# chaofengc/FeMaSR

Measured on AMD Instinct MI355X. Metric: SR output megapixels/sec at x4 (128->512), higher is better.
Workload: dtype f32 (1x1 convs / nn.Linear: every fp32 operand split EXACTLY into three bf16 terms, six partial products, fp32 accumulation on the bf16 matrix pipe - closer to fp64 than the fp32 fmaf chain, bit-identical to the CPU oracle)

## Files before the change

femasr_amd/csrc/kernels_misc.hip:

```cpp
#include "common.h"
#include "detmath.h"
#include <stdlib.h>
#include <string.h>
#include <type_traits>

namespace {

__device__ __forceinline__ float4 ld4(const float *p) { return *reinterpret_cast<const float4 *>(p); }

__device__ __forceinline__ int xcd_remap_misc(int bid, int nblk)
{
    const int q = nblk >> 3, r = nblk & 7, xcd = bid & 7, within = bid >> 3;
    return (xcd < r ? xcd * (q + 1) : r * (q + 1) + (xcd - r) * q) + within;
}

__global__ void pad_nchw_to_nhwc_kernel(const float *__restrict__ in, int B, int C, int H, int W, int Hp, int Wp,
                                        float *__restrict__ out, size_t total)
{
    for (size_t i = blockIdx.x * (size_t)blockDim.x + threadIdx.x; i < total; i += (size_t)gridDim.x * blockDim.x) {
        const int c = (int)(i % C);
        size_t r = i / C;
        const int x = (int)(r % Wp);
        r /= Wp;
        const int y = (int)(r % Hp);
// ... 149 lines not shown
    const int slabs = C >> 5, cg = C >> 5;
    int b = blockIdx.x;
    const int slab = b % slabs;
    b /= slabs;
    const int tx = b % tilesX;
    b /= tilesX;
    const int ty = b % tilesY;
    const int n = b / tilesY;
    const float *xn = x + (size_t)n * H * W * C + slab * 32 + c31;
    double S = 0.0, SS = 0.0;
#pragma unroll
    for (int q = 0; q < 4; ++q) {
        double s = 0.0, ss = 0.0;
#pragma unroll
        for (int r = 0; r < 16; ++r) {
            const int m = 32 * q + 4 * h + (r & 3) + 8 * (r >> 2);
            const int y = 8 * ty + (m >> 4), xx = 16 * tx + (m & 15);
            if (y < H && xx < W) {
                const double d = (double)xn[((size_t)y * W + xx) * C];
                s = s + d;
                ss = __builtin_fma(d, d, ss);
            }
        }
        s = s + __shfl_xor(s, 32, 64);
        ss = ss + __shfl_xor(ss, 32, 64);
        for (int d = 1; d < cg; d <<= 1) {
            s = s + __shfl_xor(s, d, 64);
            ss = ss + __shfl_xor(ss, d, 64);
        }
        if (q == 0) { S = s; SS = ss; } else { S = S + s; SS = SS + ss; }
    }
    const int ch = slab * 32 + c31;
    if (lane < 32 && (ch & (cg - 1)) == 0) {
        double *dst = part + ((((size_t)n * tilesY + ty) * tilesX + tx) * 32 + ch / cg) * 2;
        dst[0] = S;
        dst[1] = SS;
    }
}

__global__ __launch_bounds__(64) void gn_finalize_partials_kernel(const double *__restrict__ part, int tiles, int H, int W, int C, int G,
                                                                  const float *__restrict__ gamma, const float *__restrict__ beta,
                                                                  float eps, float *__restrict__ a, float *__restrict__ b)
{
    const int n = blockIdx.x / G, g = blockIdx.x % G, lane = threadIdx.x, cg = C / G;
    const double *src = part + ((size_t)n * tiles * G + g) * 2;
    double S = 0.0, SS = 0.0;
    for (int t = lane; t < tiles; t += 64) {
        S += src[(size_t)t * G * 2];
        SS += src[(size_t)t * G * 2 + 1];
    }
#pragma unroll
    for (int sft = 32; sft >= 1; sft >>= 1) {
        S += __shfl_xor(S, sft, 64);
        SS += __shfl_xor(SS, sft, 64);
    }
    const double N = (double)H * (double)W * (double)cg;
    const double mean = S / N;
    double var = SS / N - mean * mean;
    if (var < 0.0) var = 0.0;
    const float rstd = 1.0f / sqrtf((float)var + eps);
    const float meanf = (float)mean;
    if (lane < cg) {
        const int c = g * cg + lane;
        const float ac = rstd * gamma[c];
        a[n * C + c] = ac;
        b[n * C + c] = __builtin_fmaf(-meanf, ac, beta[c]);
    }
}

__global__ void gn_silu_apply_kernel(const float *__restrict__ x, int C, long long hw, const float *__restrict__ a, const float *__restrict__ b,
                                     float *__restrict__ y, size_t total4)
{
    const int c4n = C >> 2;
    for (size_t i = blockIdx.x * (size_t)blockDim.x + threadIdx.x; i < total4; i += (size_t)gridDim.x * blockDim.x) {
        const int c4 = (int)(i % c4n);
        const size_t n = (i / c4n) / (size_t)hw;
        const float4 v = ld4(x + 4 * i), ga = ld4(a + n * C + 4 * c4), gb = ld4(b + n * C + 4 * c4);
        float4 o;
        o.x = det_silu(__builtin_fmaf(v.x, ga.x, gb.x));
        o.y = det_silu(__builtin_fmaf(v.y, ga.y, gb.y));
        o.z = det_silu(__builtin_fmaf(v.z, ga.z, gb.z));
        o.w = det_silu(__builtin_fmaf(v.w, ga.w, gb.w));
        *reinterpret_cast<float4 *>(y + 4 * i) = o;
    }
}

__device__ __forceinline__ float wave_tree_sum(float p)
{
#pragma unroll
    for (int s = 32; s >= 1; s >>= 1) p = p + __shfl_xor(p, s, 64);
    return p;
}

__global__ void ln_stats_kernel(const float *__restrict__ x, long long rows, float eps, float *__restrict__ stats)
{
    const long long row = (long long)blockIdx.x * (blockDim.x >> 6) + (threadIdx.x >> 6);
    if (row >= rows) return;
    const int lane = threadIdx.x & 63;
    const float4 v = ld4(x + row * 256 + lane * 4);
    float s = v.x;
    s = s + v.y;
    s = s + v.z;
    s = s + v.w;
    const float mean = wave_tree_sum(s) * (1.0f / 256.0f);
    float d = v.x - mean;
    float q = d * d;
    d = v.y - mean;
    q = __builtin_fmaf(d, d, q);
    d = v.z - mean;
    q = __builtin_fmaf(d, d, q);
    d = v.w - mean;
    q = __builtin_fmaf(d, d, q);
    const float var = wave_tree_sum(q) * (1.0f / 256.0f);
    if (lane == 0) {
        stats[2 * row] = mean;
        stats[2 * row + 1] = 1.0f / sqrtf(var + eps);
    }
}

__global__ void layernorm_kernel(const float *__restrict__ x, long long rows, const float *__restrict__ gamma,
                                 const float *__restrict__ beta, float eps, float *__restrict__ y)
{
    const long long row = (long long)blockIdx.x * (blockDim.x >> 6) + (threadIdx.x >> 6);
    if (row >= rows) return;
    const int lane = threadIdx.x & 63;
    const float4 v = ld4(x + row * 256 + lane * 4);
    float s = v.x;
    s = s + v.y;
    s = s + v.z;
    s = s + v.w;
    const float mean = wave_tree_sum(s) * (1.0f / 256.0f);
    float d = v.x - mean;
    float q = d * d;
    d = v.y - mean;
    q = __builtin_fmaf(d, d, q);
    d = v.z - mean;
    q = __builtin_fmaf(d, d, q);
    d = v.w - mean;
    q = __builtin_fmaf(d, d, q);
    const float var = wave_tree_sum(q) * (1.0f / 256.0f);
    const float rstd = 1.0f / sqrtf(var + eps);
    const float4 g = ld4(gamma + lane * 4), b = ld4(beta + lane * 4);
    float4 o;
    o.x = __builtin_fmaf((v.x - mean) * rstd, g.x, b.x);
    o.y = __builtin_fmaf((v.y - mean) * rstd, g.y, b.y);
    o.z = __builtin_fmaf((v.z - mean) * rstd, g.z, b.z);
    o.w = __builtin_fmaf((v.w - mean) * rstd, g.w, b.w);
    *reinterpret_cast<float4 *>(y + row * 256 + lane * 4) = o;
}

constexpr int ATT_HD = 32, ATT_N = 64;
typedef float att_f32x16 __attribute__((ext_vector_type(16)));

template <int UNITS>
__global__ __launch_bounds__(64, 2) void window_attention_reg_kernel(const float *__restrict__ qkv, int B, int H, int W, int C,
                                                                     int heads, int shift, const float *__restrict__ table,
                                                                     float *__restrict__ out, int total)
{
    __shared__ float Ts[UNITS][232];
    const int lane = threadIdx.x, c = lane & 31, hf = lane >> 5;
    const int nwx = W >> 3, nwy = H >> 3;
    struct Unit { int h, wx, wy, n; };
    auto unit_of = [&](int bid) {
        Unit g;
        g.h = bid % heads;
        bid /= heads;
        g.wx = bid % nwx;
        bid /= nwx;
        g.wy = bid % nwy;
        g.n = bid / nwy;
        return g;
    };
    Unit gs[UNITS];
    bool has[UNITS];
#pragma unroll
    for (int u = 0; u < UNITS; ++u) {
        const int bid = (int)blockIdx.x * UNITS + u;
        has[u] = bid < total;
        gs[u] = unit_of(has[u] ? bid : total - 1);
        for (int i = lane; i < 225; i += 64) Ts[u][i] = table[i * heads + gs[u].h];
    }
    const float scale = 0.17677669529663687f;
    auto rowtok = [&](const Unit &g, int iy) { int y = g.wy * 8 + iy + shift; if (y >= H) y -= H; return y * W; };
    auto coltok = [&](const Unit &g, int ix) { int x = g.wx * 8 + ix + shift; if (x >= W) x -= W; return x; };
    auto qb = [&](const Unit &g) { return qkv + (size_t)g.n * H * W * 3 * C + g.h * ATT_HD; };

    float ak[2][16], bq[2][16];
    auto load_qk = [&](const Unit &g) {
        const float *qbase = qb(g);
#pragma unroll
        for (int tI = 0; tI < 2; ++tI) {
            const int w = 32 * tI + c;
            const unsigned tok = (unsigned)(rowtok(g, w >> 3) + coltok(g, w & 7));
            const float *kp = qbase + tok * (unsigned)(3 * C) + C, *qp = qbase + tok * (unsigned)(3 * C);
#pragma unroll
            for (int d4 = 0; d4 < 8; ++d4) {
                const float4 kv = ld4(kp + 4 * d4), qv = ld4(qp + 4 * d4);
                ak[tI][2 * d4] = hf ? kv.y : kv.x;
                ak[tI][2 * d4 + 1] = hf ? kv.w : kv.z;
                bq[tI][2 * d4] = (hf ? qv.y : qv.x) * scale;
                bq[tI][2 * d4 + 1] = (hf ? qv.w : qv.z) * scale;
            }
        }
    };
    load_qk(gs[0]);
#pragma unroll
    for (int u = 0; u < UNITS; ++u) {
        if (!has[u]) break;
        const Unit g = gs[u];
        const float *qbase = qb(g);
        float *obase = out + (size_t)g.n * H * W * C + g.h * ATT_HD;
        const bool masked = shift > 0 && (g.wy == nwy - 1 || g.wx == nwx - 1);
        att_f32x16 sc[2][2];
#pragma unroll
        for (int tj = 0; tj < 2; ++tj)
#pragma unroll
            for (int ti = 0; ti < 2; ++ti)
#pragma unroll
                for (int r = 0; r < 16; ++r) sc[tj][ti][r] = 0.f;
#pragma unroll
        for (int st = 0; st < 16; ++st)
#pragma unroll
            for (int tj = 0; tj < 2; ++tj)
#pragma unroll
                for (int ti = 0; ti < 2; ++ti) sc[tj][ti] = __builtin_amdgcn_mfma_f32_32x32x2f32(ak[tj][st], bq[ti][st], sc[tj][ti], 0, 0, 0);

        float vf[2][16];
        {
            const float *vb = qbase + 2 * C + c;
            unsigned cto[4];
#pragma unroll
            for (int e = 0; e < 4; ++e) cto[e] = (unsigned)coltok(g, e + 4 * hf) * (unsigned)(3 * C);
#pragma unroll
            for (int tj = 0; tj < 2; ++tj)
#pragma unroll
                for (int r = 0; r < 16; ++r) {
                    const unsigned ro = (unsigned)__builtin_amdgcn_readfirstlane(rowtok(g, (r >> 2) + 4 * tj)) * (unsigned)(3 * C);
                    vf[tj][r] = vb[ro + cto[r & 3]];
                }
        }
        if (u + 1 < UNITS && has[u + 1 < UNITS ? u + 1 : u]) load_qk(gs[u + 1 < UNITS ? u + 1 : u]);
#pragma unroll
        for (int ti = 0; ti < 2; ++ti) {
            const int i = 32 * ti + c, iy = i >> 3, ix = i & 7;
            const int tb = (iy + 7) * 15 + ix + 7 - 4 * hf;
            unsigned rowdiff = 0, coldiff = 0;
            if (masked) {
                const int ysi = g.wy * 8 + iy, xsi = g.wx * 8 + ix;
                const int ryi = ysi < H - 8 ? 0 : (ysi < H - shift ? 1 : 2), rxi = xsi < W - 8 ? 0 : (xsi < W - shift ? 1 : 2);
#pragma unroll
                for (int q = 0; q < 8; ++q) {
                    const int ysj = g.wy * 8 + q, xsj = g.wx * 8 + q;
                    const int ryj = ysj < H - 8 ? 0 : (ysj < H - shift ? 1 : 2), rxj = xsj < W - 8 ? 0 : (xsj < W - shift ? 1 : 2);
                    rowdiff |= (ryj != ryi ? 1u : 0u) << q;
                    coldiff |= (rxj != rxi ? 1u : 0u) << q;
                }
                coldiff >>= 4 * hf;
            }
            float m = -INFINITY;
#pragma unroll
            for (int tj = 0; tj < 2; ++tj)
#pragma unroll
                for (int r = 0; r < 16; ++r) {
                    const int jy = (r >> 2) + 4 * tj, jxl = r & 3;
                    float a1 = sc[tj][ti][r] + Ts[u][tb - 15 * jy - jxl];
                    if (masked) a1 = a1 + ((((rowdiff >> jy) | (coldiff >> jxl)) & 1u) ? -100.0f : 0.0f);
                    sc[tj][ti][r] = a1;
                    m = a1 > m ? a1 : m;
                }
            {
                const float mo = __shfl_xor(m, 32, 64);
                m = mo > m ? mo : m;
            }
            float part = 0.f;
#pragma unroll
            for (int tj = 0; tj < 2; ++tj)
#pragma unroll
                for (int r = 0; r < 16; r += 2) {
                    const det_f32x2 e = det_expf2(det_f32x2{sc[tj][ti][r] - m, sc[tj][ti][r + 1] - m});
                    sc[tj][ti][r] = e[0];
                    sc[tj][ti][r + 1] = e[1];
                    part = part + e[0];
                    part = part + e[1];
                }
            const float other = __shfl_xor(part, 32, 64);
            const float rinv = 1.0f / (hf ? other + part : part + other);
#pragma unroll
            for (int tj = 0; tj < 2; ++tj) sc[tj][ti] = sc[tj][ti] * rinv;
        }

        att_f32x16 oc[2];
#pragma unroll
        for (int ti = 0; ti < 2; ++ti)
#pragma unroll
            for (int r = 0; r < 16; ++r) oc[ti][r] = 0.f;
#pragma unroll
        for (int tj = 0; tj < 2; ++tj)
#pragma unroll
            for (int r = 0; r < 16; ++r)
#pragma unroll
                for (int ti = 0; ti < 2; ++ti) oc[ti] = __builtin_amdgcn_mfma_f32_32x32x2f32(sc[tj][ti][r], vf[tj][r], oc[ti], 0, 0, 0);

        {
            float *ob = obase + c;
            unsigned cto[4];
#pragma unroll
            for (int e = 0; e < 4; ++e) cto[e] = (unsigned)coltok(g, e + 4 * hf) * (unsigned)C;
#pragma unroll
            for (int ti = 0; ti < 2; ++ti)
#pragma unroll
                for (int r = 0; r < 16; ++r) {
                    const unsigned ro = (unsigned)__builtin_amdgcn_readfirstlane(rowtok(g, (r >> 2) + 4 * ti)) * (unsigned)C;
                    ob[ro + cto[r & 3]] = oc[ti][r];
                }
        }
    }
}

__global__ void row_sqsum_kernel(const float *__restrict__ x, long long rows, int D, float *__restrict__ out)
{
    const long long r = (long long)blockIdx.x * blockDim.x + threadIdx.x;
    if (r >= rows) return;
    const float *p = x + r * D;
    float acc = 0.f;
    for (int c = 0; c < D; c += 4) {
        const float4 v = ld4(p + c);
        acc = __builtin_fmaf(v.x, v.x, acc);
        acc = __builtin_fmaf(v.y, v.y, acc);
        acc = __builtin_fmaf(v.z, v.z, acc);
        acc = __builtin_fmaf(v.w, v.w, acc);
    }
    out[r] = acc;
}

__global__ void vq_finalize_kernel(const float *__restrict__ z, long long M, int D, const float *__restrict__ cb,
                                   const float *__restrict__ part, int nblk, int n_e, long long *__restrict__ idx,
                                   float *__restrict__ zq)
{
    const long long row = (long long)blockIdx.x * (blockDim.x >> 6) + (threadIdx.x >> 6);
    if (row >= M) return;
    const int lane = threadIdx.x & 63;
    const float *pp = part + (size_t)row * nblk * 2;
    float bd = pp[0];
    int bi = __float_as_int(pp[1]);
    for (int b = 1; b < nblk; ++b) {
        const float d = pp[2 * b];
        const int i = __float_as_int(pp[2 * b + 1]);
        if (d < bd || (d == bd && i < bi)) { bd = d; bi = i; }
    }
    bi = bi < 0 ? 0 : (bi >= n_e ? n_e - 1 : bi);
    if (lane == 0) idx[row] = (long long)bi;
    const float *e = cb + (size_t)bi * D;
    const float *zr = z + (size_t)row * D;
    float *o = zq + (size_t)row * D;
    for (int c = lane * 4; c < D; c += 256) {
        const float4 zv = ld4(zr + c), ev = ld4(e + c);
        float4 r;
        r.x = zv.x + (ev.x - zv.x);
        r.y = zv.y + (ev.y - zv.y);
        r.z = zv.z + (ev.z - zv.z);
        r.w = zv.w + (ev.w - zv.w);
        *reinterpret_cast<float4 *>(o + c) = r;
    }
}

__global__ void codebook_gather_kernel(const long long *__restrict__ idx, long long M, int D, const float *__restrict__ cb,
                                       int n_e, float *__restrict__ zq)
{
    const long long row = (long long)blockIdx.x * (blockDim.x >> 6) + (threadIdx.x >> 6);
    if (row >= M) return;
    const int lane = threadIdx.x & 63;
    long long i = idx[row];
    i = i < 0 ? 0 : (i >= n_e ? n_e - 1 : i);
    for (int c = lane * 4; c < D; c += 256)
        *reinterpret_cast<float4 *>(zq + (size_t)row * D + c) = ld4(cb + (size_t)i * D + c);
}

__global__ void repack_oihw_kernel(const float *__restrict__ in, int O, int I, int kh, int kw, float *__restrict__ out,
                                   size_t total)
{
    const bool blocked = (I % 32) == 0;
    const int K = I * kh * kw, NT32 = (O + 31) / 32;
    for (size_t i = blockIdx.x * (size_t)blockDim.x + threadIdx.x; i < total; i += (size_t)gridDim.x * blockDim.x) {
        const int kk = (int)(i & 15), lane = (int)((i >> 4) & 63);
        const size_t rest = i >> 10;
        const int ntile = (int)(rest % NT32), q = (int)(rest / NT32);
        const int k = q * 32 + kk * 2 + (lane >> 5), o = ntile * 32 + (lane & 31);
        float v = 0.f;
        if (k < K && o < O) {
            int ci, x, y;
            if (blocked) {
                const int cl = k % 32;
                int r = k / 32;
                x = r % kw;
                r /= kw;
                y = r % kh;
                ci = (r / kh) * 32 + cl;
            } else {
                ci = k % I;
                const int r = k / I;
                x = r % kw;
                y = r / kw;
            }
            v = in[(((size_t)o * I + ci) * kh + y) * kw + x];
        }
        out[i] = v;
    }
}

__global__ void repack_up2_kernel(const float *__restrict__ in, int O, int I, float *__restrict__ out, size_t per_phase)
{
    const int K = I * 4, NT32 = (O + 31) / 32;
    for (size_t i = blockIdx.x * (size_t)blockDim.x + threadIdx.x; i < 4 * per_phase; i += (size_t)gridDim.x * blockDim.x) {
        const int ph = (int)(i / per_phase);
        const size_t e = i - (size_t)ph * per_phase;
        const int kk = (int)(e & 15), lane = (int)((e >> 4) & 63);
        const size_t rest = e >> 10;
        const int ntile = (int)(rest % NT32), q = (int)(rest / NT32);
        const int k = q * 32 + kk * 2 + (lane >> 5), o = ntile * 32 + (lane & 31);
        float v = 0.f;
        if (k < K && o < O) {
            const int a = ph >> 1, b = ph & 1;
            const int cl = k % 32, r = k / 32, tap = r & 3, ci = (r >> 2) * 32 + cl;
            const int ty = tap >> 1, tx = tap & 1;
            const int y0 = ty == 0 ? 0 : (a == 0 ? 1 : 2), y1 = ty == 0 ? (a == 0 ? 0 : 1) : 2;
            const int x0 = tx == 0 ? 0 : (b == 0 ? 1 : 2), x1 = tx == 0 ? (b == 0 ? 0 : 1) : 2;
            const float *w = in + ((size_t)o * I + ci) * 9;
            for (int ky = y0; ky <= y1; ++ky) {
                float row = w[ky * 3 + x0];
                for (int kx = x0 + 1; kx <= x1; ++kx) row = row + w[ky * 3 + kx];
                v = ky == y0 ? row : v + row;
            }
        }
        out[i] = v;
    }
}

__global__ void repack_compact_kernel(const float *__restrict__ in, int O, int I, int kh, int kw, float *__restrict__ out, size_t total)
{
    for (size_t i = blockIdx.x * (size_t)blockDim.x + threadIdx.x; i < total; i += (size_t)gridDim.x * blockDim.x) {
        const int o = (int)(i & 3), k = (int)(i >> 2);
        const int cl = k % 32;
        int r = k / 32;
        const int x = r % kw;
        r /= kw;
        const int y = r % kh, ci = (r / kh) * 32 + cl;
        out[i] = o < O ? in[(((size_t)o * I + ci) * kh + y) * kw + x] : 0.f;
    }
}

__global__ void image_u8_to_f32_kernel(const unsigned char *__restrict__ in, int H, int W, int swap_rb,
                                       float *__restrict__ out, size_t total)
{
    for (size_t i = blockIdx.x * (size_t)blockDim.x + threadIdx.x; i < total; i += (size_t)gridDim.x * blockDim.x) {
        const int x = (int)(i % W);
        size_t r = i / W;
        const int y = (int)(r % H);
        const int c = (int)(r / H);
        const int sc = swap_rb ? 2 - c : c;
        out[i] = (float)in[((size_t)y * W + x) * 3 + sc] / 255.0f;
    }
}

__global__ void image_f32_to_u8_kernel(const float *__restrict__ in, int H, int W, int swap_rb,
                                       unsigned char *__restrict__ out, size_t total)
{
    for (size_t i = blockIdx.x * (size_t)blockDim.x + threadIdx.x; i < total; i += (size_t)gridDim.x * blockDim.x) {
        const int c = (int)(i % 3);
// ... 154 lines not shown
}

typedef float probe_f32x16 __attribute__((ext_vector_type(16)));
__global__ __launch_bounds__(256) void clock_probe_kernel(int groups, float a, float b, unsigned long long *ticks)
{
    probe_f32x16 c0 = {0}, c1 = {0}, c2 = {0}, c3 = {0};
    a += (float)(threadIdx.x & 31) * 0.03125f;
    b += (float)((threadIdx.x >> 5) & 1) * 0.25f;
    const unsigned long long t0 = __builtin_readcyclecounter();
    for (int i = 0; i < groups; ++i) {
        c0 = __builtin_amdgcn_mfma_f32_32x32x2f32(a, b, c0, 0, 0, 0);
        c1 = __builtin_amdgcn_mfma_f32_32x32x2f32(a, b, c1, 0, 0, 0);
        c2 = __builtin_amdgcn_mfma_f32_32x32x2f32(a, b, c2, 0, 0, 0);
        c3 = __builtin_amdgcn_mfma_f32_32x32x2f32(a, b, c3, 0, 0, 0);
    }
    float s = 0.f;
    for (int r = 0; r < 16; ++r) s += c0[r] + c1[r] + c2[r] + c3[r];
    const unsigned long long t1 = __builtin_readcyclecounter();
    if ((threadIdx.x & 63) == 0) ticks[blockIdx.x * 4 + (threadIdx.x >> 6)] = (t1 - t0) + (s == 12345.678f ? 1ull : 0ull);
}

extern "C" {

int femasr_pad_nchw_to_nhwc(void *stream, const float *in, int B, int C, int H, int W, int Hp, int Wp, float *out)
{
    FEMASR_REQUIRE(in && out && B > 0 && C > 0 && H > 0 && W > 0, "pad: bad args");
    FEMASR_REQUIRE(Hp >= H && Wp >= W && Hp - H <= H && Wp - W <= W, "pad: mirror pad larger than the image (%d,%d)->(%d,%d)", H, W, Hp, Wp);
    const size_t total = (size_t)B * Hp * Wp * C;
    hipLaunchKernelGGL(pad_nchw_to_nhwc_kernel, dim3(grid_for(total)), dim3(256), 0, (hipStream_t)stream, in, B, C, H, W,
                       Hp, Wp, out, total);
    FEMASR_CHECK_HIP(hipGetLastError());
    return FEMASR_OK;
}

int femasr_pad_u8hwc_to_nhwc(void *stream, const uint8_t *in, int B, int H, int W, int swap_rb, int Hp, int Wp, float *out)
{
    FEMASR_REQUIRE(in && out && B > 0 && H > 0 && W > 0 && Hp >= H && Wp >= W && Hp <= 2 * H && Wp <= 2 * W, "pad_u8: bad args");
    const size_t total = (size_t)B * Hp * Wp * 3;
    hipLaunchKernelGGL(pad_u8hwc_to_nhwc_kernel, dim3(grid_for(total)), dim3(256), 0, (hipStream_t)stream, in, B, H, W, swap_rb, Hp, Wp, out, total);
    FEMASR_CHECK_HIP(hipGetLastError());
    return FEMASR_OK;
}

int femasr_crop_nhwc_to_u8hwc(void *stream, const float *in, int B, int Hs, int Ws, int Hc, int Wc, int swap_rb, uint8_t *out)
{
    FEMASR_REQUIRE(in && out && B > 0 && Hc > 0 && Wc > 0 && Hc <= Hs && Wc <= Ws, "crop_u8: bad args");
    const size_t total = (size_t)B * Hc * Wc * 3;
    hipLaunchKernelGGL(crop_nhwc_to_u8hwc_kernel, dim3(grid_for(total)), dim3(256), 0, (hipStream_t)stream, in, B, Hs, Ws, Hc, Wc, swap_rb, out, total);
    FEMASR_CHECK_HIP(hipGetLastError());
    return FEMASR_OK;
}

int femasr_crop_nhwc_to_nchw(void *stream, const float *in, int B, int Hs, int Ws, int C, int Hc, int Wc, float *out)
{
    FEMASR_REQUIRE(in && out && B > 0 && C > 0 && Hc > 0 && Wc > 0 && Hc <= Hs && Wc <= Ws, "crop: bad args");
    const size_t total = (size_t)B * C * Hc * Wc;
    hipLaunchKernelGGL(crop_nhwc_to_nchw_kernel, dim3(grid_for(total)), dim3(256), 0, (hipStream_t)stream, in, B, Hs, Ws,
                       C, Hc, Wc, out, total);
    FEMASR_CHECK_HIP(hipGetLastError());
    return FEMASR_OK;
}

size_t femasr_gn_scratch_bytes(int B, int H, int W, int C, int G)
{
    if (B <= 0 || H <= 0 || W <= 0 || G <= 0) return 0;
    if (G == 32 && femasr_gn_fusable(C)) return (size_t)B * ((H + 7) / 8) * ((W + 15) / 16) * 32 * 2 * sizeof(double);
    return (size_t)B * H * G * 2 * sizeof(double);
}

int femasr_gn_coeffs(void *stream, const float *x, int B, int H, int W, int C, int G, const float *gamma,
                     const float *beta, float eps, float *a, float *b, void *scratch)
{
    FEMASR_REQUIRE(x && gamma && beta && a && b && scratch, "gn_coeffs: null pointer");
    FEMASR_REQUIRE(B > 0 && H > 0 && W > 0 && G > 0 && C % G == 0, "gn_coeffs: bad shape C=%d G=%d", C, G);
    const int cg = C / G;
    hipStream_t s = (hipStream_t)stream;
    double *part = (double *)scratch;
    if (G == 32 && femasr_gn_fusable(C)) {
        const int tilesX = (W + 15) / 16, tilesY = (H + 7) / 8;
        hipLaunchKernelGGL(gn_tile_partials_kernel, dim3((unsigned)((size_t)B * tilesY * tilesX * (C / 32))), dim3(64), 0, s, x, H, W, C,
                           tilesX, tilesY, part);
        FEMASR_CHECK_HIP(hipGetLastError());
        return femasr_gn_coeffs_from_partials(stream, part, B, tilesX * tilesY, H, W, C, G, gamma, beta, eps, a, b);
    }
    const size_t total = (size_t)B * H * G;
    const dim3 grid((unsigned)((total + 255) / 256)), blk(256);
    if (cg == 8 && C % 4 == 0)
        hipLaunchKernelGGL(gn_rows_kernel<8>, grid, blk, 0, s, x, B, H, W, C, G, part);
    else if (cg == 4 && C % 4 == 0)
        hipLaunchKernelGGL(gn_rows_kernel<4>, grid, blk, 0, s, x, B, H, W, C, G, part);
    else if (cg == 2)
        hipLaunchKernelGGL(gn_rows_kernel<2>, grid, blk, 0, s, x, B, H, W, C, G, part);
    else
        hipLaunchKernelGGL(gn_rows_generic_kernel, grid, blk, 0, s, x, B, H, W, C, G, cg, part);
    FEMASR_CHECK_HIP(hipGetLastError());
    FEMASR_REQUIRE(G <= 256, "gn_coeffs: at most 256 groups");
    hipLaunchKernelGGL(gn_finalize_kernel, dim3((unsigned)B), dim3(256), (size_t)GN_SLAB * G * 2 * sizeof(double), s, part, B, H, H,
                       W, C, G, gamma, beta, eps, a, b);
    FEMASR_CHECK_HIP(hipGetLastError());
    return FEMASR_OK;
}

int femasr_gn_coeffs_from_partials(void *stream, const double *part, int B, int tiles, int H, int W, int C, int G,
                                   const float *gamma, const float *beta, float eps, float *a, float *b)
{
    FEMASR_REQUIRE(part && gamma && beta && a && b && B > 0 && tiles > 0 && H > 0 && W > 0, "gn_coeffs_from_partials: bad args");
    FEMASR_REQUIRE(G == 32 && C % G == 0, "gn_coeffs_from_partials: 32 groups");
    FEMASR_REQUIRE(C / G <= 64, "gn_coeffs_from_partials: at most 64 channels per group");
    hipLaunchKernelGGL(gn_finalize_partials_kernel, dim3((unsigned)(B * G)), dim3(64), 0, (hipStream_t)stream, part, tiles, H, W, C,
                       G, gamma, beta, eps, a, b);
    FEMASR_CHECK_HIP(hipGetLastError());
    return FEMASR_OK;
}

int femasr_gn_silu_apply(void *stream, const float *x, int B, int H, int W, int C, const float *a, const float *b, float *y)
{
    FEMASR_REQUIRE(x && a && b && y && B > 0 && H > 0 && W > 0 && C > 0 && (C % 4) == 0, "gn_silu_apply: bad args (C %% 4 == 0)");
    const size_t total4 = (size_t)B * H * W * (C / 4);
    hipLaunchKernelGGL(gn_silu_apply_kernel, dim3(grid_for(total4)), dim3(256), 0, (hipStream_t)stream, x, C, (long long)H * W, a, b, y, total4);
    FEMASR_CHECK_HIP(hipGetLastError());
    return FEMASR_OK;
}

int femasr_ln_stats(void *stream, const float *x, int64_t rows, int C, float eps, float *stats)
{
    FEMASR_REQUIRE(x && stats && rows > 0, "ln_stats: bad args");
    FEMASR_REQUIRE(C == 256, "ln_stats: only C == 256 (Swin embed_dim, femasr_arch.py:115) is built, got %d", C);
    hipLaunchKernelGGL(ln_stats_kernel, dim3((unsigned)((rows + 3) / 4)), dim3(256), 0, (hipStream_t)stream, x,
                       (long long)rows, eps, stats);
    FEMASR_CHECK_HIP(hipGetLastError());
    return FEMASR_OK;
}

int femasr_layernorm(void *stream, const float *x, int64_t rows, int C, const float *gamma, const float *beta, float eps, float *y)
{
    FEMASR_REQUIRE(x && y && gamma && beta && rows > 0, "layernorm: bad args");
    FEMASR_REQUIRE(C == 256, "layernorm: only C == 256 (Swin embed_dim, femasr_arch.py:115) is built, got %d", C);
    hipLaunchKernelGGL(layernorm_kernel, dim3((unsigned)((rows + 3) / 4)), dim3(256), 0, (hipStream_t)stream, x, (long long)rows,
                       gamma, beta, eps, y);
    FEMASR_CHECK_HIP(hipGetLastError());
    return FEMASR_OK;
}

int femasr_window_attention(void *stream, const float *qkv, int B, int H, int W, int C, int heads, int shift,
                            const float *table, float *out)
{
    FEMASR_REQUIRE(qkv && table && out && B > 0, "window_attention: bad args");
    FEMASR_REQUIRE(H % 8 == 0 && W % 8 == 0 && H >= 8 && W >= 8, "window_attention: H,W must be multiples of 8 (%d,%d)", H, W);
    FEMASR_REQUIRE(heads > 0 && heads <= 8 && C == heads * ATT_HD, "window_attention: head_dim must be 32, at most 8 heads (C=%d heads=%d)", C, heads);
    FEMASR_REQUIRE(shift >= 0 && shift < 8, "window_attention: bad shift %d", shift);
    FEMASR_REQUIRE((size_t)H * W * 3 * C < ((size_t)1 << 30), "window_attention: image too large for 32-bit offsets");
    const size_t total = (size_t)B * (H / 8) * (W / 8) * heads;
    FEMASR_REQUIRE(total < ((size_t)1 << 31), "window_attention: too many (window, head) units");
    hipLaunchKernelGGL(window_attention_reg_kernel<1>, dim3((unsigned)total), dim3(64), 0, (hipStream_t)stream, qkv, B, H, W, C, heads, shift, table,
                       out, (int)total);
    FEMASR_CHECK_HIP(hipGetLastError());
    return FEMASR_OK;
}

int femasr_row_sqsum(void *stream, const float *x, int64_t rows, int D, float *out)
{
    FEMASR_REQUIRE(x && out && rows > 0 && D > 0 && D % 4 == 0, "row_sqsum: bad args");
    hipLaunchKernelGGL(row_sqsum_kernel, dim3((unsigned)((rows + 63) / 64)), dim3(64), 0, (hipStream_t)stream, x,
                       (long long)rows, D, out);
    FEMASR_CHECK_HIP(hipGetLastError());
    return FEMASR_OK;
}

int femasr_vq(void *stream, const float *z, int64_t M, int D, const float *cb, const float *cbT, const float *ee,
              int n_e, int64_t *idx, float *zq, void *scratch)
{
    FEMASR_REQUIRE(z && cb && cbT && ee && idx && zq && scratch && M > 0, "vq: bad args");
    FEMASR_REQUIRE(D % 32 == 0 && n_e % 128 == 0, "vq: needs e_dim %% 32 == 0 and n_e %% 128 == 0 (D=%d n_e=%d)", D, n_e);
    FEMASR_REQUIRE(M < (1ll << 31) - 256, "vq: too many rows");
    hipStream_t s = (hipStream_t)stream;
    float *zz = (float *)scratch;
    float *part = zz + ((M + 63) / 64) * 64;
    const int nblk = n_e / 128;
    int rc = femasr_row_sqsum(stream, z, M, D, zz);
    if (rc) return rc;
    femasr_conv_args a{};
    a.in = z; a.B = 1; a.H = (int)M; a.W = 1; a.Cin = D; a.w = cbT; a.bias = nullptr; a.Cout = n_e;
    a.ksz = 1; a.stride = 1; a.pad = 0; a.up2 = 0; a.prologue = FEMASR_PRO_NONE; a.act = 0;
    a.Ho = (int)M; a.Wo = 1;
    conv_vq_epilogue ep{zz, ee, part, nblk};
    rc = femasr_conv2d_launch(s, &a, &ep, nullptr, nullptr);
    if (rc) return rc;
    hipLaunchKernelGGL(vq_finalize_kernel, dim3((unsigned)((M + 3) / 4)), dim3(256), 0, s, z, (long long)M, D, cb, part,
                       nblk, n_e, (long long *)idx, zq);
    FEMASR_CHECK_HIP(hipGetLastError());
    return FEMASR_OK;
}

int femasr_codebook_gather(void *stream, const int64_t *idx, int64_t M, int D, const float *cb, int n_e, float *zq)
{
    FEMASR_REQUIRE(idx && cb && zq && M > 0 && D % 4 == 0 && n_e > 0, "codebook_gather: bad args");
    hipLaunchKernelGGL(codebook_gather_kernel, dim3((unsigned)((M + 3) / 4)), dim3(256), 0, (hipStream_t)stream,
                       (const long long *)idx, (long long)M, D, cb, n_e, zq);
    FEMASR_CHECK_HIP(hipGetLastError());
    return FEMASR_OK;
}

int femasr_extract_tiles(void *stream, const float *in, int B, int C, int H, int W, const int32_t *yx_dev, int n, int th, int tw, float *out)
{
    FEMASR_REQUIRE(in && yx_dev && out && B > 0 && C > 0 && n > 0 && th > 0 && tw > 0 && th <= H && tw <= W, "extract_tiles: bad args");
    const size_t total = (size_t)n * B * C * th * tw;
    hipLaunchKernelGGL(extract_tiles_kernel, dim3(grid_for(total)), dim3(256), 0, (hipStream_t)stream, in, B, C, H, W, yx_dev, n, th, tw, out, total);
    FEMASR_CHECK_HIP(hipGetLastError());
    return FEMASR_OK;
}

int femasr_paste_tiles(void *stream, const float *tiles, int B, int C, int n, int th, int tw, const int32_t *rects_dev, int hmax,
                       int Ho, int Wo, float *out)
{
    FEMASR_REQUIRE(tiles && rects_dev && out && B > 0 && C > 0 && n > 0 && th > 0 && tw > 0 && hmax > 0 && hmax <= th, "paste_tiles: bad args");
    const size_t rows = (size_t)n * B * C * hmax;
    FEMASR_REQUIRE(rows < ((size_t)1 << 31), "paste_tiles: too many rows");
    hipLaunchKernelGGL(paste_tiles_kernel, dim3((unsigned)rows), dim3(256), 0, (hipStream_t)stream, tiles, B, C, th, tw, rects_dev, n, Ho, Wo, out, hmax);
    FEMASR_CHECK_HIP(hipGetLastError());
    return FEMASR_OK;
}

int femasr_extract_tiles_u8(void *stream, const uint8_t *in, int B, int H, int W, const int32_t *yx_dev, int n, int th, int tw, uint8_t *out)
{
    FEMASR_REQUIRE(in && yx_dev && out && B > 0 && n > 0 && th > 0 && tw > 0 && th <= H && tw <= W, "extract_tiles_u8: bad args");
    const size_t total = (size_t)n * B * th * tw * 3;
    hipLaunchKernelGGL(extract_tiles_u8_kernel, dim3(grid_for(total)), dim3(256), 0, (hipStream_t)stream, in, B, H, W, yx_dev, n, th, tw, out, total);
    FEMASR_CHECK_HIP(hipGetLastError());
    return FEMASR_OK;
}

int femasr_paste_tiles_u8(void *stream, const uint8_t *tiles, int B, int n, int th, int tw, const int32_t *rects_dev, int hmax, int Ho, int Wo, uint8_t *out)
{
    FEMASR_REQUIRE(tiles && rects_dev && out && B > 0 && n > 0 && th > 0 && tw > 0 && hmax > 0 && hmax <= th, "paste_tiles_u8: bad args");
    const size_t rows = (size_t)n * B * hmax;
    FEMASR_REQUIRE(rows < ((size_t)1 << 31), "paste_tiles_u8: too many rows");
    hipLaunchKernelGGL(paste_tiles_u8_kernel, dim3((unsigned)rows), dim3(256), 0, (hipStream_t)stream, tiles, B, th, tw, rects_dev, n, Ho, Wo, out, hmax);
    FEMASR_CHECK_HIP(hipGetLastError());
    return FEMASR_OK;
}

static int blend_launch(bool u8, void *stream, const uint64_t *tile_ptrs_dev, const int32_t *geom_dev, int n, int tiles_y, int tiles_x,
                        int pitch, int B, int C, int Ho, int Wo, void *out)
{
    const char *who = u8 ? "blend_tiles_u8" : "blend_tiles";
    FEMASR_REQUIRE(tile_ptrs_dev && geom_dev && out, "%s: null pointer", who);
    FEMASR_REQUIRE(n > 0 && B > 0 && C > 0 && tiles_y > 0 && tiles_x > 0 && pitch > 0 && Ho > 0 && Wo > 0, "%s: bad sizes", who);
    FEMASR_REQUIRE((long long)tiles_y * tiles_x == n, "%s: %d tiles given for a %d x %d grid", who, n, tiles_y, tiles_x);
    FEMASR_REQUIRE(tiles_x <= 65535, "%s: more than 65535 tile columns", who);
    const size_t rows = (size_t)B * C * Ho;
    FEMASR_REQUIRE(rows < ((size_t)1 << 31), "%s: too many rows", who);
    const dim3 grid((unsigned)rows, (unsigned)tiles_x);
    if (u8)
        hipLaunchKernelGGL(blend_tiles_kernel<true>, grid, dim3(256), 0, (hipStream_t)stream, (const unsigned long long *)tile_ptrs_dev,
                           geom_dev, tiles_y, tiles_x, pitch, 1, Ho, Wo, out);
    else
        hipLaunchKernelGGL(blend_tiles_kernel<false>, grid, dim3(256), 0, (hipStream_t)stream, (const unsigned long long *)tile_ptrs_dev,
                           geom_dev, tiles_y, tiles_x, pitch, C, Ho, Wo, out);
    FEMASR_CHECK_HIP(hipGetLastError());
    return FEMASR_OK;
}

int femasr_blend_tiles(void *stream, const uint64_t *tile_ptrs_dev, const int32_t *geom_dev, int n, int tiles_y, int tiles_x, int pitch,
                       int B, int C, int Ho, int Wo, float *out)
{
    return blend_launch(false, stream, tile_ptrs_dev, geom_dev, n, tiles_y, tiles_x, pitch, B, C, Ho, Wo, out);
}

int femasr_blend_tiles_u8(void *stream, const uint64_t *tile_ptrs_dev, const int32_t *geom_dev, int n, int tiles_y, int tiles_x, int pitch,
                          int B, int Ho, int Wo, uint8_t *out)
{
    return blend_launch(true, stream, tile_ptrs_dev, geom_dev, n, tiles_y, tiles_x, pitch, B, 1, Ho, Wo, out);
}

int femasr_concat_resize(void *stream, const float *a, int Ca, const float *b, int Hb, int Wb, int Cb, int B, int H, int W, float *out)
{
    FEMASR_REQUIRE(a && b && out && B > 0 && H > 0 && W > 0 && Hb > 0 && Wb > 0, "concat_resize: bad args");
    FEMASR_REQUIRE(Ca > 0 && Cb > 0 && Ca % 4 == 0 && Cb % 4 == 0, "concat_resize: channel counts must be multiples of 4 (%d, %d)", Ca, Cb);
    const size_t total4 = (size_t)B * H * W * ((Ca + Cb) / 4);
    hipLaunchKernelGGL(concat_resize_kernel, dim3(grid_for(total4)), dim3(256), 0, (hipStream_t)stream, a, Ca, b, Hb, Wb, Cb, H, W, out,
                       total4);
    FEMASR_CHECK_HIP(hipGetLastError());
    return FEMASR_OK;
}

size_t femasr_packed_weight_floats(int O, int I, int kh, int kw)
{
    if (O <= 0 || I <= 0 || kh <= 0 || kw <= 0) return 0;
    const size_t K = (size_t)I * kh * kw;
    return ((K + 31) / 32) * (size_t)((O + 31) / 32) * 1024 + femasr_compact_weight_floats(O, I, kh, kw);
}

int femasr_repack_oihw(void *stream, const float *in, int O, int I, int kh, int kw, float *out)
{
    FEMASR_REQUIRE(in && out && O > 0 && I > 0 && kh > 0 && kw > 0, "repack: bad args");
    if (kh == 1 && kw == 1 && (I % 32) == 0) return femasr_repack_k1((hipStream_t)stream, in, O, I, out);
    const size_t tail = femasr_compact_weight_floats(O, I, kh, kw);
    const size_t total = femasr_packed_weight_floats(O, I, kh, kw) - tail;
    if (tail) {
        hipLaunchKernelGGL(repack_compact_kernel, dim3(grid_for(tail)), dim3(256), 0, (hipStream_t)stream, in, O, I, kh, kw, out + total, tail);
        FEMASR_CHECK_HIP(hipGetLastError());
    }
    hipLaunchKernelGGL(repack_oihw_kernel, dim3(grid_for(total)), dim3(256), 0, (hipStream_t)stream, in, O, I, kh, kw, out,
                       total);
    FEMASR_CHECK_HIP(hipGetLastError());
    return FEMASR_OK;
}

size_t femasr_up2_weight_floats(int O, int I)
{
    return (I % 32) == 0 ? 4 * femasr_packed_weight_floats(O, I, 2, 2) : 0;
// ... 150 lines not shown
```

Before: 70.08.

## Make window attention persistent and stage next unit's Q/K into LDS asynchronously

```diff
diff --git a/femasr_amd/csrc/kernels_misc.hip b/femasr_amd/csrc/kernels_misc.hip
--- a/femasr_amd/csrc/kernels_misc.hip
+++ b/femasr_amd/csrc/kernels_misc.hip
@@ -325,14 +325,26 @@
 constexpr int ATT_HD = 32, ATT_N = 64;
 typedef float att_f32x16 __attribute__((ext_vector_type(16)));
 
-template <int UNITS>
+constexpr int ATT_KQ = 2 * ATT_N * ATT_HD;
+constexpr int ATT_WAVES_PER_CU = 8;
+
+#ifdef FEMASR_ATT_TT
+__device__ unsigned long long *g_att_ttbuf;
+#define ATT_TT(slot) { __builtin_amdgcn_sched_barrier(0); if (lane == 0) g_att_ttbuf[((size_t)blockIdx.x * 8 + (trip < 7 ? trip : 7)) * 8 + (slot)] = __builtin_readcyclecounter(); __builtin_amdgcn_sched_barrier(0); }
+#else
+#define ATT_TT(slot) {}
+#endif
+
 __global__ __launch_bounds__(64, 2) void window_attention_reg_kernel(const float *__restrict__ qkv, int B, int H, int W, int C,
                                                                      int heads, int shift, const float *__restrict__ table,
-                                                                     float *__restrict__ out, int total)
-{
-    __shared__ float Ts[UNITS][232];
+                                                                     float *__restrict__ out, int total, int waves)
+{
+    __shared__ __attribute__((aligned(1024))) float KQ[ATT_KQ];
+    __shared__ float Ts[232];
     const int lane = threadIdx.x, c = lane & 31, hf = lane >> 5;
     const int nwx = W >> 3, nwy = H >> 3;
+    int trip = 0;
+    ATT_TT(0)
     struct Unit { int h, wx, wy, n; };
     auto unit_of = [&](int bid) {
         Unit g;
@@ -344,45 +356,58 @@
         g.n = bid / nwy;
         return g;
     };
-    Unit gs[UNITS];
-    bool has[UNITS];
-#pragma unroll
-    for (int u = 0; u < UNITS; ++u) {
-        const int bid = (int)blockIdx.x * UNITS + u;
-        has[u] = bid < total;
-        gs[u] = unit_of(has[u] ? bid : total - 1);
-        for (int i = lane; i < 225; i += 64) Ts[u][i] = table[i * heads + gs[u].h];
-    }
     const float scale = 0.17677669529663687f;
     auto rowtok = [&](const Unit &g, int iy) { int y = g.wy * 8 + iy + shift; if (y >= H) y -= H; return y * W; };
     auto coltok = [&](const Unit &g, int ix) { int x = g.wx * 8 + ix + shift; if (x >= W) x -= W; return x; };
     auto qb = [&](const Unit &g) { return qkv + (size_t)g.n * H * W * 3 * C + g.h * ATT_HD; };
 
-    float ak[2][16], bq[2][16];
-    auto load_qk = [&](const Unit &g) {
+    auto stage_qk = [&](const Unit &g) {
+        typedef __attribute__((address_space(1))) const void *gptr_t;
+        typedef __attribute__((address_space(3))) void *lptr_t;
         const float *qbase = qb(g);
+        const unsigned ct = (unsigned)coltok(g, lane >> 3) * (unsigned)(3 * C);
+        unsigned lo[2];
+#pragma unroll
+        for (int e = 0; e < 2; ++e) lo[e] = 4u * (ct + 4u * (unsigned)((lane & 7) ^ (4 * e + (lane >> 4))));
+#pragma unroll
+        for (int i = 0; i < 8; ++i) {
+            const char *qrow = reinterpret_cast<const char *>(qbase + (unsigned)__builtin_amdgcn_readfirstlane(rowtok(g, i)) * (unsigned)(3 * C));
+            const char *krow = reinterpret_cast<const char *>(qbase + (unsigned)__builtin_amdgcn_readfirstlane(rowtok(g, i)) * (unsigned)(3 * C) + C);
+            __builtin_amdgcn_global_load_lds((gptr_t)(krow + lo[i & 1]), (lptr_t)(KQ + i * 256), 16, 0, 0);
+            __builtin_amdgcn_global_load_lds((gptr_t)(qrow + lo[i & 1]), (lptr_t)(KQ + ATT_N * ATT_HD + i * 256), 16, 0, 0);
+        }
+    };
+
+    int u = (int)blockIdx.x;
+    Unit g = unit_of(u);
+    float tv[4];
+#pragma unroll
+    for (int k = 0; k < 4; ++k) tv[k] = table[(lane + 64 * k < 225 ? lane + 64 * k : 224) * heads + g.h];
+    stage_qk(g);
+#pragma unroll
+    for (int k = 0; k < 4; ++k)
+        if (lane + 64 * k < 225) Ts[lane + 64 * k] = tv[k];
+    ATT_TT(1)
+    __builtin_amdgcn_s_waitcnt(0x0F70);
+    for (;; ++trip) {
+        if (trip) ATT_TT(0)
+        const float *qbase = qb(g);
+        float *obase = out + (size_t)g.n * H * W * C + g.h * ATT_HD;
+        float ak[2][16], bq[2][16];
 #pragma unroll
         for (int tI = 0; tI < 2; ++tI) {
-            const int w = 32 * tI + c;
-            const unsigned tok = (unsigned)(rowtok(g, w >> 3) + coltok(g, w & 7));
-            const float *kp = qbase + tok * (unsigned)(3 * C) + C, *qp = qbase + tok * (unsigned)(3 * C);
+            const float *kr = KQ + (32 * tI + c) * ATT_HD, *qr = kr + ATT_N * ATT_HD;
 #pragma unroll
             for (int d4 = 0; d4 < 8; ++d4) {
-                const float4 kv = ld4(kp + 4 * d4), qv = ld4(qp + 4 * d4);
+                const int p = 4 * (d4 ^ ((c >> 1) & 7));
+                const float4 kv = ld4(kr + p), qv = ld4(qr + p);
                 ak[tI][2 * d4] = hf ? kv.y : kv.x;
                 ak[tI][2 * d4 + 1] = hf ? kv.w : kv.z;
                 bq[tI][2 * d4] = (hf ? qv.y : qv.x) * scale;
                 bq[tI][2 * d4 + 1] = (hf ? qv.w : qv.z) * scale;
             }
         }
-    };
-    load_qk(gs[0]);
-#pragma unroll
-    for (int u = 0; u < UNITS; ++u) {
-        if (!has[u]) break;
-        const Unit g = gs[u];
-        const float *qbase = qb(g);
-        float *obase = out + (size_t)g.n * H * W * C + g.h * ATT_HD;
+        ATT_TT(2)
         const bool masked = shift > 0 && (g.wy == nwy - 1 || g.wx == nwx - 1);
         att_f32x16 sc[2][2];
 #pragma unroll
@@ -398,21 +423,26 @@
 #pragma unroll
                 for (int ti = 0; ti < 2; ++ti) sc[tj][ti] = __builtin_amdgcn_mfma_f32_32x32x2f32(ak[tj][st], bq[ti][st], sc[tj][ti], 0, 0, 0);
 
+        const bool more = total - u > waves;
+        Unit gn = g;
+        if (more) {
+            gn = unit_of(u + waves);
+            stage_qk(gn);
+        }
+        ATT_TT(3)
         float vf[2][16];
         {
-            const float *vb = qbase + 2 * C + c;
             unsigned cto[4];
 #pragma unroll
-            for (int e = 0; e < 4; ++e) cto[e] = (unsigned)coltok(g, e + 4 * hf) * (unsigned)(3 * C);
+            for (int e = 0; e < 4; ++e) cto[e] = 4u * ((unsigned)coltok(g, e + 4 * hf) * (unsigned)(3 * C) + (unsigned)c);
 #pragma unroll
             for (int tj = 0; tj < 2; ++tj)
 #pragma unroll
                 for (int r = 0; r < 16; ++r) {
-                    const unsigned ro = (unsigned)__builtin_amdgcn_readfirstlane(rowtok(g, (r >> 2) + 4 * tj)) * (unsigned)(3 * C);
-                    vf[tj][r] = vb[ro + cto[r & 3]];
+                    const float *vr = qbase + 2 * C + (unsigned)__builtin_amdgcn_readfirstlane(rowtok(g, (r >> 2) + 4 * tj)) * (unsigned)(3 * C);
+                    vf[tj][r] = *reinterpret_cast<const float *>(reinterpret_cast<const char *>(vr) + cto[r & 3]);
                 }
         }
-        if (u + 1 < UNITS && has[u + 1 < UNITS ? u + 1 : u]) load_qk(gs[u + 1 < UNITS ? u + 1 : u]);
 #pragma unroll
         for (int ti = 0; ti < 2; ++ti) {
             const int i = 32 * ti + c, iy = i >> 3, ix = i & 7;
@@ -436,7 +466,7 @@
 #pragma unroll
                 for (int r = 0; r < 16; ++r) {
                     const int jy = (r >> 2) + 4 * tj, jxl = r & 3;
-                    float a1 = sc[tj][ti][r] + Ts[u][tb - 15 * jy - jxl];
+                    float a1 = sc[tj][ti][r] + Ts[tb - 15 * jy - jxl];
                     if (masked) a1 = a1 + ((((rowdiff >> jy) | (coldiff >> jxl)) & 1u) ? -100.0f : 0.0f);
                     sc[tj][ti][r] = a1;
                     m = a1 > m ? a1 : m;
@@ -461,6 +491,7 @@
 #pragma unroll
             for (int tj = 0; tj < 2; ++tj) sc[tj][ti] = sc[tj][ti] * rinv;
         }
+        ATT_TT(4)
 
         att_f32x16 oc[2];
 #pragma unroll
@@ -474,19 +505,27 @@
 #pragma unroll
                 for (int ti = 0; ti < 2; ++ti) oc[ti] = __builtin_amdgcn_mfma_f32_32x32x2f32(sc[tj][ti][r], vf[tj][r], oc[ti], 0, 0, 0);
 
+        __builtin_amdgcn_s_waitcnt(0x0F70);
+#ifdef FEMASR_ATT_TT
+        asm volatile("" : "+v"(oc[0]), "+v"(oc[1]));
+#endif
+        ATT_TT(5)
         {
-            float *ob = obase + c;
             unsigned cto[4];
 #pragma unroll
-            for (int e = 0; e < 4; ++e) cto[e] = (unsigned)coltok(g, e + 4 * hf) * (unsigned)C;
+            for (int e = 0; e < 4; ++e) cto[e] = 4u * ((unsigned)coltok(g, e + 4 * hf) * (unsigned)C + (unsigned)c);
 #pragma unroll
             for (int ti = 0; ti < 2; ++ti)
 #pragma unroll
                 for (int r = 0; r < 16; ++r) {
-                    const unsigned ro = (unsigned)__builtin_amdgcn_readfirstlane(rowtok(g, (r >> 2) + 4 * ti)) * (unsigned)C;
-                    ob[ro + cto[r & 3]] = oc[ti][r];
+                    float *orow = obase + (unsigned)__builtin_amdgcn_readfirstlane(rowtok(g, (r >> 2) + 4 * ti)) * (unsigned)C;
+                    *reinterpret_cast<float *>(reinterpret_cast<char *>(orow) + cto[r & 3]) = oc[ti][r];
                 }
         }
+        ATT_TT(6)
+        if (!more) break;
+        u += waves;
+        g = gn;
     }
 }
 
@@ -947,11 +986,26 @@
     FEMASR_REQUIRE((size_t)H * W * 3 * C < ((size_t)1 << 30), "window_attention: image too large for 32-bit offsets");
     const size_t total = (size_t)B * (H / 8) * (W / 8) * heads;
     FEMASR_REQUIRE(total < ((size_t)1 << 31), "window_attention: too many (window, head) units");
-    hipLaunchKernelGGL(window_attention_reg_kernel<1>, dim3((unsigned)total), dim3(64), 0, (hipStream_t)stream, qkv, B, H, W, C, heads, shift, table,
-                       out, (int)total);
-    FEMASR_CHECK_HIP(hipGetLastError());
-    return FEMASR_OK;
-}
+    static const int resident = [] {
+        int dev = 0, cus = 0;
+        if (hipGetDevice(&dev) == hipSuccess && hipDeviceGetAttribute(&cus, hipDeviceAttributeMultiprocessorCount, dev) == hipSuccess && cus > 0)
+            return cus * ATT_WAVES_PER_CU;
+        return 256 * ATT_WAVES_PER_CU;
+    }();
+    const int waves = resident / heads > 0 ? resident / heads * heads : heads;
+    const unsigned grid = (unsigned)(total < (size_t)waves ? total : (size_t)waves);
+    hipLaunchKernelGGL(window_attention_reg_kernel, dim3(grid), dim3(64), 0, (hipStream_t)stream, qkv, B, H, W, C, heads, shift, table,
+                       out, (int)total, waves);
+    FEMASR_CHECK_HIP(hipGetLastError());
+    return FEMASR_OK;
+}
+
+#ifdef FEMASR_ATT_TT
+int femasr_debug_attention_ttbuf(unsigned long long *dev_buf)
+{
+    return (int)hipMemcpyToSymbol(HIP_SYMBOL(g_att_ttbuf), &dev_buf, sizeof(dev_buf));
+}
+#endif
 
 int femasr_row_sqsum(void *stream, const float *x, int64_t rows, int D, float *out)
 {
```

Result: no change. 70.39, median of 6 (+0.4%).
